# zhoujun-7/VPHO

Hardware: AMD Instinct MI355X
Metric: eval images/sec (bs=64, sample_num=100, steps=50); MPJPE delta vs ref (higher is better)
Workload: dtype f32; 1 GPU; vpho_net.forward(mode=predict), README eval config (BASELINE.json configs[1]); per_gpu_batch=64, sample_num=100, sampling_steps=50, topk_hand=30, topk_obj=10, crop=256x256, pipeline_depth=3, parallelism=dp1, score_mfma=f32, conv_mfma=f32, winograd_3x3=True

## Files before the change

vpho_amd/csrc/conv_igemm.hip:

```cpp
#include "common.h"
#include "../../include/vpho_hip.h"
#include <cstdlib>
#include <algorithm>

VPHO_STAMP_DECL(conv)

namespace {

#ifndef CONV_ABLATE
#define CONV_ABLATE 0
#endif
constexpr int BK = 32;
constexpr int LDS_LD = BK + 4;
constexpr int GLDS_PRE_MAX = 512;

struct Geo {
    vpho_conv_desc d;
    int M, K, tiles_m, tiles_n, ntiles;
    int w_ld;
    long long x_zs, w_zs, y_zs;
    long long b_zs, r_zs, x2_zs, pre_zs, ru_zs;
    int y_linear, r_linear, vec_epilogue;
    int uni;
    int dbg;
};

__device__ __forceinline__ void advance_group(vpho_conv_desc& d, const Geo& g, const unsigned by) {
    d.x += by * g.x_zs; d.w += by * g.w_zs; d.y += by * g.y_zs;
    if (d.bias) d.bias += by * g.b_zs;
    if (d.res) d.res += by * g.r_zs;
    if (d.x2) d.x2 += by * g.x2_zs;
    if (d.in_scale) { d.in_scale += by * g.pre_zs; d.in_shift += by * g.pre_zs; }
    if (d.res_up) d.res_up += by * g.ru_zs;
}

template <int BM, int BN, int WM, int WN, int VEC>
__global__ __launch_bounds__(64 * WM * WN) void conv_igemm_kernel(const Geo g) {
    constexpr int NT = 64 * WM * WN;
    constexpr int TM = BM / (32 * WM), TN = BN / (32 * WN);
    constexpr int KQN = 8 / VEC;
    constexpr int ROWS = NT / KQN;
    constexpr int A_LD = (BM + ROWS - 1) / ROWS, B_LD = (BN + ROWS - 1) / ROWS;
    constexpr bool A_PART = BM < ROWS, B_PART = BN < ROWS;
    static_assert(TM >= 1 && TN >= 1, "tile too small for the wave layout");
    __shared__ __attribute__((aligned(16))) float smem[2 * (BM + BN) * LDS_LD];

    vpho_conv_desc d = g.d;
    advance_group(d, g, blockIdx.y);
    int per_xcd = gridDim.x >> 3, ntiles = g.ntiles, M_live = g.M;
    if (d.row_map) {
        M_live = min(*d.row_count, g.M);
        ntiles = (M_live + BM - 1) / BM * g.tiles_n;
        per_xcd = (ntiles + 7) >> 3;
        if ((int)(blockIdx.x >> 3) >= per_xcd) return;
    }
    const int lb = (blockIdx.x & 7) * per_xcd + (blockIdx.x >> 3);
    if (lb >= ntiles) return;
    const int tile_n = lb % g.tiles_n, tile_m = lb / g.tiles_n;
    const int m0 = tile_m * BM, n0 = tile_n * BN;

    const int tid = threadIdx.x, lane = tid & 63, wave = tid >> 6;
    const int li = lane & 31, lh = lane >> 5;
    const int wm = wave / WN, wn = wave % WN;
    const int kq = tid % KQN, lrow = tid / KQN;

    long long a_off[A_LD];
// ... 598 lines not shown
            float* R = smem;
            if (lane < V_PER_ROW) {
                *reinterpret_cast<f32x4*>(R + (wave * 4 + 0) * BN + 4 * lane) = st0;
                *reinterpret_cast<f32x4*>(R + (wave * 4 + 1) * BN + 4 * lane) = st1;
                *reinterpret_cast<f32x4*>(R + (wave * 4 + 2) * BN + 4 * lane) = piv;
                *reinterpret_cast<f32x4*>(R + (wave * 4 + 3) * BN + 4 * lane) = f32x4{cnt, cnt, cnt, cnt};
            }
            __syncthreads();
            if (d.bn_x) {
                if (tid < 2 * BN) {
                    const int pl = tid / BN, c = tid - pl * BN;
                    float t = R[pl * BN + c];
#pragma unroll
                    for (int k = 1; k < NWAVES; ++k) t += R[(k * 4 + pl) * BN + c];
                    if (n0 + c < d.Cout) d.stats[((long long)tile_m * BN_STAT_PLANES + pl) * d.Cout + n0 + c] = t;
                }
            } else if (tid < BN) {
                const int c = tid;
                ShiftSums t{R[2 * BN + c], R[c], R[BN + c], R[3 * BN + c]};
#pragma unroll
                for (int k = 1; k < NWAVES; ++k) t = shift_sums_add(t, ShiftSums{R[(k * 4 + 2) * BN + c], R[(k * 4) * BN + c], R[(k * 4 + 1) * BN + c], R[(k * 4 + 3) * BN + c]});
                if (n0 + c < d.Cout) store_bn_row(d.stats + (long long)tile_m * BN_STAT_PLANES * d.Cout + n0 + c, d.Cout, t);
            }
        }
        VPHO_STAMP_AT(4);
        VPHO_STAMP_WRITE(conv, blockIdx.x);
        return;
    }
    const int row_base = m0 + wm * (BM / WM) + 4 * lh, col_base = n0 + wn * (BN / WN) + li;
#pragma unroll
    for (int j = 0; j < TN; ++j) {
        const int col = col_base + j * 32;
        if (col >= d.Cout) continue;
        const float bv = d.bias ? d.bias[col] : 0.f;
#pragma unroll
        for (int i = 0; i < TM; ++i) {
#pragma unroll
            for (int e = 0; e < 16; ++e) {
                const int row = row_base + i * 32 + (e & 3) + 8 * (e >> 2);
                if (row >= M_live) continue;
                long long yoff, ro;
                offsets(row, yoff, ro);
                float v = acc[i][j][e] + bv;
                if (d.res) v += d.res[ro + col];
                v = v > 0.f ? v : v * d.out_slope;
                if (d.gate) v = d.gate[yoff + col] > 0.f ? v : v * d.gate_slope;
                d.y[yoff + col] = v;
            }
        }
    }
}

#define VPHO_WAIT_VM(n) asm volatile("s_waitcnt vmcnt(%0)" :: "n"(n) : "memory")
template <int BM, int BN, int WM, int WN, bool STATS>
__device__ __forceinline__ void conv_pers_body(const Geo& g) {
    constexpr int NT = 64 * WM * WN, NW = WM * WN;
    constexpr int TM = BM / (32 * WM), TN = BN / (32 * WN);
    constexpr int ROWS = NT / 8;
    constexpr int A_LD = BM / ROWS, B_LD = BN / ROWS, NF = A_LD + B_LD;
    static_assert(TM >= 1 && TN >= 1 && A_LD >= 1 && B_LD >= 1 && ROWS % 16 == 0 && BN / WN <= 64, "tile/wave layout");
    constexpr int TILE = (BM + BN) * BK;
    constexpr int EPI = 8 * 32;
    constexpr int NIT = TM * 4 * TN;
    __shared__ __attribute__((aligned(1024))) float smem[2 * TILE + NW * EPI + 2 * BN];
    VPHO_STAMP_INIT();

    vpho_conv_desc d = g.d;
    advance_group(d, g, blockIdx.y);
    const int tid = threadIdx.x, lane = tid & 63, wave = __builtin_amdgcn_readfirstlane(tid >> 6);
    const int li = lane & 31, lh = lane >> 5;
    const int wm = wave / WN, wn = wave % WN;
    const int lrow = wave * 8 + (lane >> 3);
    const int kq = (lane & 7) ^ ((lrow >> 1) & 7);
    const int ohw = d.OH * d.OW;
    const __amdgpu_buffer_rsrc_t xu = __builtin_amdgcn_make_buffer_rsrc(const_cast<float*>(d.x), 0, 0xFFFFFFF0u, 0x00020000);
    const __amdgpu_buffer_rsrc_t wr = __builtin_amdgcn_make_buffer_rsrc(const_cast<float*>(d.w), 0, 0xFFFFFFF0u, 0x00020000);
    const __amdgpu_buffer_rsrc_t x2r = __builtin_amdgcn_make_buffer_rsrc(const_cast<float*>(d.x2 ? d.x2 : d.x), 0, 0xFFFFFFF0u, 0x00020000);
    const __amdgpu_buffer_rsrc_t yr = __builtin_amdgcn_make_buffer_rsrc(d.y, 0, 0xFFFFFFF0u, 0x00020000);
    const __amdgpu_buffer_rsrc_t rr = __builtin_amdgcn_make_buffer_rsrc(const_cast<float*>(d.res ? d.res : d.y), 0, 0xFFFFFFF0u, 0x00020000);
    const __amdgpu_buffer_rsrc_t br = __builtin_amdgcn_make_buffer_rsrc(const_cast<float*>(d.bias ? d.bias : d.w), 0, 0xFFFFFFF0u, 0x00020000);
    typedef __attribute__((address_space(3))) void* lds_ptr;

    const int xcd = blockIdx.x & 7, nslot = gridDim.x >> 3, per_xcd = (g.ntiles + 7) >> 3;
    int lt = blockIdx.x >> 3;
    auto tile_at = [&](int t, int& m0, int& n0) -> bool {
        const int lb = xcd * per_xcd + t;
        if (t >= per_xcd || lb >= g.ntiles) return false;
        const int tile_m = lb / g.tiles_n, tile_n = lb - tile_m * g.tiles_n;
        m0 = tile_m * BM; n0 = tile_n * BN;
        return true;
    };
    int m0, n0;
    if (!tile_at(lt, m0, n0)) return;

    int u_voff[A_LD], u_boff[B_LD], u_voff2[A_LD], bias_off;
    auto setup = [&](int m0_, int n0_) {
#pragma unroll
        for (int j = 0; j < A_LD; ++j) {
            const int m = m0_ + lrow + ROWS * j;
            u_voff[j] = -1; u_voff2[j] = -1;
            if (m < g.M) {
                const int n = m / ohw, rem = m - n * ohw;
                const int oy = rem / d.OW, ox = rem - oy * d.OW;
                u_voff[j] = (int)((((long long)(n * d.H + oy * d.stride) * d.W + ox * d.stride) * d.x_ld) * 4 + 16 * kq);
                if (d.x2) u_voff2[j] = (int)((((long long)(n * d.H2 + oy * d.stride2) * d.W2 + ox * d.stride2) * d.x2_ld) * 4 + 16 * kq);
            }
        }
#pragma unroll
        for (int j = 0; j < B_LD; ++j) {
            const int n = n0_ + lrow + ROWS * j;
            u_boff[j] = n < d.Cout ? (int)(((long long)n * g.w_ld + 4 * kq) * 4) : -1;
        }
        const int bc = n0_ + wn * (BN / WN) + lane;
        bias_off = (d.bias && lane < BN / WN && bc < d.Cout) ? bc * 4 : -1;
    };
    auto fill = [&](int buf, int kt, int tp) {
        float* As = smem + buf * TILE + wave * 8 * BK;
        float* Bs = smem + buf * TILE + BM * BK + wave * 8 * BK;
        if (d.x2 && kt * BK >= d.Cin) {
            const int c2 = (kt * BK - d.Cin) * 4;
#pragma unroll
            for (int j = 0; j < A_LD; ++j) {
                const int vo = u_voff2[j];
                __builtin_amdgcn_raw_ptr_buffer_load_lds(x2r, (lds_ptr)(As + ROWS * j * BK), 16, vo, c2, 0, 0);
            }
        } else {
            const int c1 = kt * BK * 4;
#pragma unroll
            for (int j = 0; j < A_LD; ++j) {
                const int vo = u_voff[j];
                __builtin_amdgcn_raw_ptr_buffer_load_lds(xu, (lds_ptr)(As + ROWS * j * BK), 16, vo, c1, 0, 0);
            }
        }
        const int koff = kt * BK * 4;
#pragma unroll
        for (int j = 0; j < B_LD; ++j) {
            const int bo = u_boff[j];
            __builtin_amdgcn_raw_ptr_buffer_load_lds(wr, (lds_ptr)(Bs + ROWS * j * BK), 16, bo, koff, 0, 0);
        }
        if (kt == 0) {
            const int bo = bias_off;
            __builtin_amdgcn_raw_ptr_buffer_load_lds(br, (lds_ptr)(smem + 2 * TILE + NW * EPI + tp * BN + wn * (BN / WN)), 4, bo, 0, 0, 0);
        }
    };

    const int nk = (g.K + BK - 1) / BK;
    const int sw = (li >> 1) & 7;
    f32x16 acc[TM][TN];
    auto compute = [&](int kt) {
        const int buf = kt & 1;
        const float* As = smem + buf * TILE + (wm * (BM / WM) + li) * BK;
        const float* Bs = smem + buf * TILE + BM * BK + (wn * (BN / WN) + li) * BK;
#pragma unroll
        for (int kk = 0; kk < BK / 8; ++kk) {
            const int ch = ((2 * kk + lh) ^ sw) * 4;
            f32x4 a[TM], b[TN];
#pragma unroll
            for (int i = 0; i < TM; ++i) a[i] = *reinterpret_cast<const f32x4*>(As + i * 32 * BK + ch);
#pragma unroll
            for (int j = 0; j < TN; ++j) b[j] = *reinterpret_cast<const f32x4*>(Bs + j * 32 * BK + ch);
#pragma unroll
            for (int q = 0; q < 4; ++q)
#pragma unroll
                for (int i = 0; i < TM; ++i)
#pragma unroll
                    for (int j = 0; j < TN; ++j)
                        acc[i][j] = __builtin_amdgcn_mfma_f32_32x32x2f32(a[i][q], b[j][q], acc[i][j], 0, 0, 0);
        }
    };

    float* Cw = smem + 2 * TILE + wave * EPI;
    const int er = lane >> 3, ec = (lane & 7) * 4;
    auto item_off = [&](int m0_, int n0_, int i, int gq, int j, int& yo, int& ro) {
        const int row = m0_ + wm * (BM / WM) + i * 32 + 8 * gq + er, col = n0_ + wn * (BN / WN) + j * 32 + ec;
        yo = ro = -1;
        if (row < g.M && col < d.Cout) {
            long long y_, r_;
            if (g.y_linear && g.r_linear) { y_ = (long long)row * d.y_sx; r_ = (long long)row * d.r_sx; }
            else {
                const int n = row / ohw, rem = row - n * ohw;
                const int oy = rem / d.OW, ox = rem - oy * d.OW;
                y_ = n * d.y_sn + oy * d.y_sy + ox * d.y_sx; r_ = n * d.r_sn + oy * d.r_sy + ox * d.r_sx;
            }
            yo = (int)((y_ + col) * 4);
            if (d.res) ro = (int)((r_ + col) * 4);
        }
    };

    constexpr bool stats_on = STATS;
    static_assert(4 * (BN / WN) <= EPI && BN <= NT, "stats layout");
    auto flush_stats = [&](int m0_, int n0_) {
        if (tid < BN) {
            const int c = tid;
            const int wn_c = c / (BN / WN), cc = c - wn_c * (BN / WN);
            const float* q = smem + 2 * TILE + wn_c * EPI + cc;
            constexpr int PL = BN / WN;
            ShiftSums t{q[2 * PL], q[0], q[PL], q[3 * PL]};
#pragma unroll
            for (int w = 1; w < WM; ++w) {
                const float* r = q + w * WN * EPI;
                t = shift_sums_add(t, ShiftSums{r[2 * PL], r[0], r[PL], r[3 * PL]});
            }
            if (n0_ + c < d.Cout) store_bn_row(d.stats + (long long)(m0_ / BM) * BN_STAT_PLANES * d.Cout + n0_ + c, d.Cout, t);
        }
    };
    int pm0 = 0, pn0 = 0;

    int tp = 0;
    setup(m0, n0);
    fill(0, 0, tp);
    if (nk > 1) fill(1, 1, tp);
    VPHO_STAMP_AT(1);
    bool first = true;
    while (true) {
        if (nk > 1) { if (first) VPHO_WAIT_VM(NF); else VPHO_WAIT_VM(NF + NIT); }
        else        { if (first) VPHO_WAIT_VM(0);  else VPHO_WAIT_VM(NIT); }
        VPHO_BARRIER_LDS_ONLY();
        if (stats_on && !first) flush_stats(pm0, pn0);
        if (first) VPHO_STAMP_AT(2);
        VPHO_PRIO_MAIN();
#pragma unroll
        for (int i = 0; i < TM; ++i)
#pragma unroll
            for (int j = 0; j < TN; ++j)
#pragma unroll
                for (int e = 0; e < 16; ++e) acc[i][j][e] = 0.f;
        for (int kt = 0; kt + 1 < nk; ++kt) {
            if (kt > 0) fill((kt & 1) ^ 1, kt + 1, tp);
            compute(kt);
            VPHO_SYNC_LDS_DMA();
        }
        f32x4 rv[NIT];
#pragma unroll
        for (int i = 0; i < TM; ++i)
#pragma unroll
            for (int gq = 0; gq < 4; ++gq)
#pragma unroll
                for (int j = 0; j < TN; ++j) {
                    int yo, ro;
                    item_off(m0, n0, i, gq, j, yo, ro);
                    rv[(i * 4 + gq) * TN + j] = __builtin_bit_cast(f32x4, __builtin_amdgcn_raw_buffer_load_b128(rr, ro, 0, 0));
                }
        __builtin_amdgcn_sched_barrier(0);
        compute(nk - 1);
        VPHO_SYNC_LDS_DMA();
#pragma unroll
        for (int k = 0; k < NIT; ++k) asm volatile("" :: "v"(rv[k]));
        VPHO_PRIO_REST();
        if (first) VPHO_STAMP_AT(3);
        const int em0 = m0, en0 = n0, etp = tp;
        lt += nslot;
        const bool more = tile_at(lt, m0, n0);
        if (more) {
            tp ^= 1;
            setup(m0, n0);
            fill(0, 0, tp);
            if (nk > 1) fill(1, 1, tp);
        }
        const float* Bq = smem + 2 * TILE + NW * EPI + etp * BN + wn * (BN / WN) + ec;
        f32x4 st0[TN], st1[TN], piv[TN];
#pragma unroll
        for (int j = 0; j < TN; ++j) { st0[j] = f32x4{0.f, 0.f, 0.f, 0.f}; st1[j] = st0[j]; piv[j] = st0[j]; }
#pragma unroll
        for (int i = 0; i < TM; ++i)
#pragma unroll
            for (int gq = 0; gq < 4; ++gq)
#pragma unroll
                for (int j = 0; j < TN; ++j) {
#pragma unroll
                    for (int e4 = 0; e4 < 4; ++e4) Cw[(e4 + 4 * lh) * 32 + li] = acc[i][j][4 * gq + e4];
                    int yo, ro;
                    item_off(em0, en0, i, gq, j, yo, ro);
                    const f32x4 v = *reinterpret_cast<const f32x4*>(Cw + er * 32 + ec);
                    const f32x4 bq = *reinterpret_cast<const f32x4*>(Bq + j * 32);
                    const f32x4 r = rv[(i * 4 + gq) * TN + j];
                    f32x4 o;
#pragma unroll
                    for (int k = 0; k < 4; ++k) { const float t = v[k] + bq[k] + r[k]; o[k] = t > 0.f ? t : t * d.out_slope; }
                    __builtin_amdgcn_raw_buffer_store_b128(__builtin_bit_cast(__attribute__((__vector_size__(4 * sizeof(unsigned)))) unsigned, o), yr, yo, 0, 0);
                    if (stats_on) {
                        if (i == 0 && gq == 0) {
#pragma unroll
                            for (int k = 0; k < 4; ++k) piv[j][k] = __shfl(o[k], lane & 7);
                        }
#pragma unroll
                        for (int k = 0; k < 4; ++k) { const float u = yo != -1 ? o[k] - piv[j][k] : 0.f; st0[j][k] += u; st1[j][k] += u * u; }
                    }
                }
        if (stats_on) {
            const float n = (float)max(0, min(BM / WM, g.M - (em0 + wm * (BM / WM))));
            static_assert(TM * 32 == BM / WM, "a wave's rows are one block");
#pragma unroll
            for (int j = 0; j < TN; ++j) {
#pragma unroll
                for (int k = 0; k < 4; ++k) { st0[j][k] = sum_lane_bits_345(st0[j][k]); st1[j][k] = sum_lane_bits_345(st1[j][k]); }
                if (lane < 8) {
                    *reinterpret_cast<f32x4*>(Cw + j * 32 + ec) = st0[j];
                    *reinterpret_cast<f32x4*>(Cw + (BN / WN) + j * 32 + ec) = st1[j];
                    *reinterpret_cast<f32x4*>(Cw + 2 * (BN / WN) + j * 32 + ec) = piv[j];
                    *reinterpret_cast<f32x4*>(Cw + 3 * (BN / WN) + j * 32 + ec) = f32x4{n, n, n, n};
                }
            }
            pm0 = em0; pn0 = en0;
        }
        if (first) { VPHO_STAMP_AT(4); }
        first = false;
        if (!more) break;
    }
    if (stats_on) { VPHO_BARRIER_LDS_ONLY(); flush_stats(pm0, pn0); }
    VPHO_STAMP_WRITE(conv, blockIdx.x);
}
template <int BM, int BN, int WM, int WN>
__global__ __launch_bounds__(64 * WM * WN, 4) void conv_igemm_pers_kernel(const Geo g) { conv_pers_body<BM, BN, WM, WN, false>(g); }
template <int BM, int BN, int WM, int WN>
__global__ __launch_bounds__(64 * WM * WN, 4) void conv_igemm_pers_bn_kernel(const Geo g) { conv_pers_body<BM, BN, WM, WN, true>(g); }

typedef __bf16 cbf16x8 __attribute__((ext_vector_type(8)));
constexpr int SBK = 16;

__device__ __forceinline__ void conv_split3(const f32x4& x0, const f32x4& x1, cbf16x8& h, cbf16x8& m, cbf16x8& l) {
#pragma unroll
    for (int e = 0; e < 8; ++e) {
        const float x = e < 4 ? x0[e] : x1[e - 4];
        const __bf16 hb = (__bf16)x;
        const float r1 = x - (float)hb;
        const __bf16 mb = (__bf16)r1;
        const float r2 = r1 - (float)mb;
        h[e] = hb; m[e] = mb; l[e] = (__bf16)r2;
    }
}

template <int BM, int BN, int WM, int WN, int TERMS>
__global__ __launch_bounds__(64 * WM * WN) void conv_igemm_split_kernel(const Geo g) {
    constexpr int NT = 64 * WM * WN, NW = WM * WN;
    constexpr int TM = BM / (32 * WM), TN = BN / (32 * WN);
    constexpr int A_ROWS = NW * 16;
    constexpr int A_LD = BM / A_ROWS;
    constexpr int B_ROWS = NW * 32;
    constexpr int B_PASSES = (3 * BN + B_ROWS - 1) / B_ROWS;
    static_assert(TM >= 1 && TN >= 1 && A_LD >= 1 && BM % A_ROWS == 0, "tile/wave layout");
    constexpr int A_FLOATS = BM * SBK, PLANE_FLOATS = BN * SBK / 2;
    constexpr int TILE = A_FLOATS + 3 * PLANE_FLOATS;
    constexpr int EPI_FLOATS = BM * BN;
    __shared__ __attribute__((aligned(1024))) float smem[(2 * TILE > EPI_FLOATS) ? 2 * TILE : EPI_FLOATS];

    vpho_conv_desc d = g.d;
    int per_xcd = gridDim.x >> 3, ntiles = g.ntiles, M_live = g.M;
    if (d.row_map) {
        M_live = min(*d.row_count, g.M);
        ntiles = (M_live + BM - 1) / BM * g.tiles_n;
        per_xcd = (ntiles + 7) >> 3;
        if ((int)(blockIdx.x >> 3) >= per_xcd) return;
    }
    const int lb = (blockIdx.x & 7) * per_xcd + (blockIdx.x >> 3);
    if (lb >= ntiles) return;
    const int tile_n = lb % g.tiles_n, tile_m = lb / g.tiles_n;
    const int m0 = tile_m * BM, n0 = tile_n * BN;

    const int tid = threadIdx.x, lane = tid & 63, wave = __builtin_amdgcn_readfirstlane(tid >> 6);
    const int li = lane & 31, lh = lane >> 5;
    const int wm = wave / WN, wn = wave % WN;
    const int ohw = d.OH * d.OW;

    const long long pad_shift = ((long long)d.pad_y * d.W + d.pad_x) * d.x_ld;
    const __amdgpu_buffer_rsrc_t xu = __builtin_amdgcn_make_buffer_rsrc(
        reinterpret_cast<void*>(reinterpret_cast<uintptr_t>(d.x) - (uintptr_t)(pad_shift * 4)), 0, 0xFFFFFFF0u, 0x00020000);
    const int arow = wave * 16 + (lane >> 2);
    int a_iy0[A_LD], a_ix0[A_LD], u_voff[A_LD];
// ... 265 lines not shown
                if (d.bn_x && d.bn_gamma) g.d.gate = nullptr;
            } else {
                g.d.stats = nullptr;
                if (d.bn_x) { if (!d.gate) { stats_failed = true; return; } g.d.bn_x = nullptr; }
            }
        }
        hipLaunchKernelGGL(kernel, dim3((g.ntiles + 7) / 8 * 8, ny), dim3(threads), 0, s, g);
    };
    static const int no_glds = getenv("VPHO_CONV_NO_GLDS") ? atoi(getenv("VPHO_CONV_NO_GLDS")) : 0;
    const double x_extent = 4.0 * (((double)d.N * d.H * d.W - 1) * d.x_ld + d.Cin + (double)(ny - 1) * (double)g.x_zs);
    const double w_extent = 4.0 * (((double)d.Cout - 1) * g.w_ld + g.K + (double)(ny - 1) * (double)g.w_zs);
    VPHO_REQUIRE(x_extent < 3.9e9 && w_extent < 3.9e9 && g.x_zs >= 0 && g.w_zs >= 0,
                 "vpho_conv2d_nhwc_f32: input (%.2f GB) and weights (%.2f GB) must each stay below 3.9 GB", x_extent * 1e-9, w_extent * 1e-9);
    static const int no_uni = getenv("VPHO_CONV_NO_UNI") ? atoi(getenv("VPHO_CONV_NO_UNI")) : 0;
    g.uni = (d.Cin % BK == 0 && d.pad_y >= 0 && d.pad_x >= 0 && !no_uni) ? 1 : 0;
    const bool pre_on_read = d.in_scale != nullptr && g.uni && d.KH == 1 && d.KW == 1 && d.pad_y == 0 && d.pad_x == 0 && d.Cin <= GLDS_PRE_MAX;
    const bool glds = (d.in_scale == nullptr || pre_on_read) && (!no_glds || d.res_up != nullptr || d.x2 != nullptr || d.bn_x != nullptr);
    stats_kernel = glds && variant != 128;
    VPHO_REQUIRE(!d.x2 || (g.uni && variant != 128), "vpho_conv2d_nhwc_f32: x2 is served by the direct-to-LDS kernels with wave-uniform taps only");
    VPHO_REQUIRE(!d.res_up || variant != 128, "vpho_conv2d_nhwc_f32: res_up is not served by the forced register-staged tile");
    const bool split_ok = d.w_planes != nullptr && (d.plane_terms == 6 || d.plane_terms == 9) && d.in_scale == nullptr && splits == 1 && !d.gate &&
                          d.Cin % SBK == 0 && g.vec_epilogue && d.pad_y >= 0 && d.pad_x >= 0 && g.w_ld == g.K &&
                          ((uintptr_t)d.w_planes & 15) == 0 && 6.0 * d.Cout * g.K < 3.9e9;
    if (split_ok) {
        const bool x9 = d.plane_terms == 9;
        switch (variant) {
            case 128: case 1288:
                if (x9) launch(conv_igemm_split_kernel<128, 128, 4, 2, 9>, 128, 128, 512, vpho::PROF_CONV128);
                else    launch(conv_igemm_split_kernel<128, 128, 4, 2, 6>, 128, 128, 512, vpho::PROF_CONV128);
                break;
            case 12864:
                if (x9) launch(conv_igemm_split_kernel<128, 64, 4, 2, 9>, 128, 64, 512, vpho::PROF_CONV128x64);
                else    launch(conv_igemm_split_kernel<128, 64, 4, 2, 6>, 128, 64, 512, vpho::PROF_CONV128x64);
                break;
            default:
                if (x9) launch(conv_igemm_split_kernel<64, 64, 2, 2, 9>, 64, 64, 256, vpho::PROF_CONV64);
                else    launch(conv_igemm_split_kernel<64, 64, 2, 2, 6>, 64, 64, 256, vpho::PROF_CONV64);
                break;
        }
        return vpho::check_launch("conv_igemm_split_kernel");
    }
    {
        const char* pe = getenv("VPHO_CONV_PERS");
        const int pers = pe ? atoi(pe) : 1;
        static int slots_of[64] = {0};
        int dev = 0;
        VPHO_HIP(hipGetDevice(&dev));
        int& slots = slots_of[dev & 63];
        if (!slots) {
            hipDeviceProp_t prop;
            VPHO_HIP(hipGetDeviceProperties(&prop, dev));
            slots = 2 * prop.multiProcessorCount;
        }
        const double y_extent = 4.0 * ((double)(d.N - 1) * d.y_sn + (double)(d.OH - 1) * d.y_sy + (double)(d.OW - 1) * d.y_sx + d.Cout);
        const double r_extent = d.res ? 4.0 * ((double)(d.N - 1) * d.r_sn + (double)(d.OH - 1) * d.r_sy + (double)(d.OW - 1) * d.r_sx + d.Cout) : 0.0;
        const bool simple = d.KH == 1 && d.KW == 1 && d.pad_y == 0 && d.pad_x == 0;
        const bool ok = pers && variant == 1288 && glds && !pre_on_read && d.in_scale == nullptr && g.uni && simple && g.vec_epilogue && !d.row_map && !d.res_up &&
                        !d.gate && !d.bn_x && splits == 1 && y_extent < 3.9e9 && r_extent < 3.9e9 && d.y_sn >= 0 && d.y_sy >= 0 && d.y_sx >= 0 &&
                        (!d.x2 || 4.0 * d.N * d.H2 * d.W2 * (double)d.x2_ld < 3.9e9);
        if (ok && (big_tiles > slots || pers >= 2)) {
            vpho::ProfScope prof(vpho::PROF_CONV128, s, flops, bytes);
            g.tiles_m = (int)((M + 127) / 128); g.tiles_n = (d.Cout + 127) / 128;
            g.ntiles = g.tiles_m * g.tiles_n;
            if (d.stats) {
                if (stats_shape && g.tiles_m <= d.stats_cap) *d.stats_rows = g.tiles_m; else g.d.stats = nullptr;
            }
            const int grid = (int)std::min<long long>((g.ntiles + 7) / 8 * 8, std::max(8, slots / groups / 8 * 8));
            if (g.d.stats) hipLaunchKernelGGL((conv_igemm_pers_bn_kernel<128, 128, 4, 2>), dim3(grid, groups), dim3(512), 0, s, g);
            else hipLaunchKernelGGL((conv_igemm_pers_kernel<128, 128, 4, 2>), dim3(grid, groups), dim3(512), 0, s, g);
            return vpho::check_launch("conv_igemm_pers_kernel");
        }
    }
    switch (variant) {
        case 128:  launch(conv_igemm_kernel<128, 128, 2, 2, 1>, 128, 128, 256, vpho::PROF_CONV128); break;
        case 1288:
            if (glds && pre_on_read) launch(conv_igemm_glds_kernel<128, 128, 4, 2, true>, 128, 128, 512, vpho::PROF_CONV128);
            else if (glds) launch(conv_igemm_glds_kernel<128, 128, 4, 2>, 128, 128, 512, vpho::PROF_CONV128);
            else      launch(conv_igemm_kernel<128, 128, 4, 2, 1>, 128, 128, 512, vpho::PROF_CONV128);
            break;
        case 12864:
            if (glds && pre_on_read) launch(conv_igemm_glds_kernel<128, 64, 4, 2, true>, 128, 64, 512, vpho::PROF_CONV128x64);
            else if (glds) launch(conv_igemm_glds_kernel<128, 64, 4, 2>, 128, 64, 512, vpho::PROF_CONV128x64);
            else      launch(conv_igemm_kernel<128, 64, 4, 2, 1>, 128, 64, 512, vpho::PROF_CONV128x64);
            break;
        default:
            if (glds && pre_on_read) launch(conv_igemm_glds_kernel<64, 64, 2, 2, true>, 64, 64, 256, vpho::PROF_CONV64);
            else if (glds) launch(conv_igemm_glds_kernel<64, 64, 2, 2>, 64, 64, 256, vpho::PROF_CONV64);
            else      launch(conv_igemm_kernel<64, 64, 2, 2, 1>, 64, 64, 256, vpho::PROF_CONV64);
            break;
    }
    if (stats_failed)
        return vpho::fail("vpho_conv2d_nhwc_f32: bn_x: the launch needs %d partial rows (stats_cap %d) or runs a kernel without the BatchNorm epilogue (tile %d)",
                          g.tiles_m, d.stats_cap, variant);
    return vpho::check_launch("conv_igemm_kernel");
}
```

vpho_amd/ops.py:

```python
import ctypes as C
import os

import torch

_HERE = os.path.dirname(os.path.abspath(__file__))
LIB_PATH = os.environ.get('VPHO_HIP_LIB') or os.path.join(_HERE, 'libvpho_hip.so')

if not os.path.exists(LIB_PATH):
    raise ImportError(f'{LIB_PATH} is missing: build the HIP extension first (python -m vpho_amd.build or '
                      f'__graft_entry__.build()); vpho_amd has no CPU fallback')
lib = C.CDLL(LIB_PATH)
lib.vpho_last_error.restype = C.c_char_p
lib.vpho_abi_version.restype = C.c_int
ABI_VERSION = 13
if lib.vpho_abi_version() != ABI_VERSION:
    raise ImportError(f'{LIB_PATH} implements ABI version {lib.vpho_abi_version()}, this binding expects {ABI_VERSION}: rebuild the '
                      f'extension (python -m vpho_amd.build --force)')
lib.vpho_obj_metrics_workspace_bytes.restype = C.c_longlong
lib.vpho_obj_metrics_multi_workspace_bytes.restype = C.c_longlong
lib.vpho_bn_workspace_bytes.restype = C.c_longlong
lib.vpho_conv2d_wgrad_workspace_bytes.restype = C.c_longlong
lib.vpho_mha_bwd_workspace_bytes.restype = C.c_longlong
lib.vpho_infer_record_bytes.restype = C.c_longlong
lib.vpho_hand_obj_intersection_workspace_bytes.restype = C.c_longlong
# ... 114 lines not shown
            assert N % G == 0, (N, G)
            N //= G
    cin = x_ld if cin is None else cin
    cout = w.shape[-2]
    assert split is not None or w.shape[-1] == kh * kw * cin + (0 if x2 is None else x2.shape[-1]), (w.shape, kh, kw, cin)
    py = pad if pad_y is None else pad_y
    px = pad if pad_x is None else pad_x
    if out_hw is None:
        OH, OW = (H + 2 * py - kh) // stride + 1, (W + 2 * px - kw) // stride + 1
    else:
        OH, OW = out_hw
    d = ConvDesc()
    d.x, d.w, d.bias = _addr(x), _addr(w), _addr(bias)
    d.in_scale, d.in_shift, d.res = _addr(in_scale), _addr(in_shift), _addr(res)
    for t in (x, w, bias, in_scale, in_shift, res):
        _ptr(t, torch.float32)
    if rows is not None:
        assert out_view is None and res is None and gate is None and rows.shape == (N, OH, OW) and (res_up is None or rows_scatter)
        if out is None:
            out = torch.empty((N, OH, OW, cout) if rows_scatter else (N * OH * OW, cout), device=x.device, dtype=torch.float32)
        _ptr(out, torch.float32)
        ld = out.shape[-1]
        d.y, d.y_sx, d.y_sy, d.y_sn = out.data_ptr(), ld, (ld * OW if rows_scatter else 0), (ld * OW * OH if rows_scatter else 0)
        d.rows_scatter = 1 if rows_scatter else 0
        d.row_map, d.row_count = rows.row_map.data_ptr(), rows.count.data_ptr()
        d.rows_hint = int(rows.count.item()) if _prof_on else 0
        ret = out
    elif out_view is not None:
        yt, d.y_sn, d.y_sy, d.y_sx, off = out_view
        _ptr(yt, torch.float32)
        d.y = yt.data_ptr() + 4 * off
        ret = yt
        if gate is not None:
            assert gate[0].shape == yt.shape and gate[0].is_contiguous() and yt.is_contiguous()
            d.gate, d.gate_slope = _ptr(gate[0], torch.float32).value + 4 * off, gate[1]
    else:
        if out is None:
            out = torch.empty((G * N, OH, OW, cout), device=x.device, dtype=torch.float32)
        _ptr(out, torch.float32)
        assert out.shape[0] == G * N
        ld = out.shape[-1]
        d.y, d.y_sx, d.y_sy, d.y_sn = out.data_ptr(), ld, ld * OW, ld * OW * OH
        ret = out
        if gate is not None:
            assert gate[0].shape == out.shape
            d.gate, d.gate_slope = _ptr(gate[0], torch.float32).value, gate[1]
    if res is not None:
        assert res.shape == (G * N, OH, OW, cout)
        d.r_sx, d.r_sy, d.r_sn = cout, cout * OW, cout * OW * OH
    if x2 is not None:
        assert kh == kw == 1 and rows is None and split is None and in_scale is None and x2.shape[0] == (N if (G == 1 or x2_shared) else G * N) and x2.is_contiguous()
        d.x2, d.Cin2, d.x2_ld, d.stride2, d.H2, d.W2 = _ptr(x2, torch.float32).value, x2.shape[3], x2.shape[3], stride2, x2.shape[1], x2.shape[2]
    if res_up is not None:
        assert res is None and res_up.shape[0] == G * N and res_up.shape[3] == cout and res_up.is_contiguous()
        d.res_up, d.ru_H, d.ru_W, d.ru_ld = _ptr(res_up, torch.float32).value, res_up.shape[1], res_up.shape[2], res_up.shape[3]
    if G > 1:
        assert in_scale is None or (in_scale.shape == (G, cin) and in_shift.shape == (G, cin) and in_scale.is_contiguous() and in_shift.is_contiguous())
        d.groups = G
        d.x_group = 0 if x_shared else N * H * W * x_ld
        d.w_group, d.bias_group, d.y_group = w.shape[1] * w.shape[2], cout, (ret.numel() // G if out_view is not None else N * OH * OW * ret.shape[-1])
        d.res_group = N * OH * OW * cout
        d.x2_group = 0 if (x2 is None or x2_shared) else N * x2.shape[1] * x2.shape[2] * x2.shape[3]
        d.pre_group = cin
        d.ru_group = 0 if res_up is None else N * res_up.shape[1] * res_up.shape[2] * res_up.shape[3]
    d.N, d.H, d.W, d.Cin, d.x_ld = N, H, W, cin, x_ld
    d.Cout, d.KH, d.KW, d.stride, d.pad_y, d.pad_x, d.OH, d.OW = cout, kh, kw, stride, py, px, OH, OW
    d.in_slope, d.out_slope = in_slope, out_slope
    if split is not None:
        d.splits, d.w_ld, d.x_split, d.w_split, d.y_split = split
    terms = getattr(_conv_split, 'terms', 0)
    if terms and G == 1 and split is None and in_scale is None and gate is None and res_up is None and x2 is None and cin % 16 == 0 and w.is_contiguous() and w.shape[1] == kh * kw * cin:
        planes = _planes_of(w)
        d.w_planes, d.plane_terms = planes.data_ptr(), terms
    rows_out = None
    if bn is not None and FUSE_BN and G == 1 and split is None and rows is None and in_scale is None and (out_view is None or bn.parts > 1) and not d.w_planes and cout % 4 == 0:
        cap = (N * OH * OW + 63) // 64
        if bn.stats is None:
            bn.stats = torch.empty((cap * bn.parts, BN_STAT_PLANES, cout), device=x.device, dtype=torch.float32)
        base = bn.rows
        assert base + cap <= bn.stats.shape[0] and bn.stats.shape[2] == cout
        rows_out = C.c_int(0)
        d.stats, d.stats_cap, d.stats_rows = bn.stats.data_ptr() + base * BN_STAT_PLANES * cout * 4, cap, C.cast(C.pointer(rows_out), C.c_void_p)
        if bn.x is not None:
            assert gate is not None and bn.x.shape == ret.shape and bn.x.is_contiguous() and ret.is_contiguous()
            bx = _ptr(bn.x, torch.float32).value + (4 * out_view[4] if out_view is not None else 0)
            if bn.stored_gate:
                d.bn_x, d.bn_mean, d.bn_invstd = bx, _ptr(bn.mean, torch.float32).value, _ptr(bn.invstd, torch.float32).value
            else:
                d.bn_x = bx
                d.bn_mean, d.bn_invstd, d.bn_gamma, d.bn_beta = (_ptr(t, torch.float32).value for t in (bn.mean, bn.invstd, bn.gamma, bn.beta))
    elif bn is not None:
        bn.failed = True
    _check(lib.vpho_conv2d_nhwc_f32(C.byref(d), _stream()))
    if rows_out is not None:
        bn.calls += 1
        if rows_out.value == 0:
            bn.failed = True
        bn.rows += rows_out.value
    return ret


def conv3x3(x, w, bias=None, out_slope=1.0, winograd=True, rows=None, groups=1, x_shared=False):
    N, H, W, x_ld = x.shape
    cout, k9 = w.shape[-2:]
    cin = k9 // 9
    if not winograd or H % 2 or W % 2 or cin % 16 or cout % 64 or x_ld != cin:
        return conv2d_nhwc(x, w, bias, kh=3, kw=3, pad=1, out_slope=out_slope, rows=rows, groups=groups, x_shared=x_shared)
# ... 1351 lines not shown
```

Measured before the change: 2104 images/s.

## Route row-gathered and upsampled-residual 1x1 convs through persistent 128x64 kernel

Adds a GATHER variant of the persistent implicit-GEMM conv body. It reads a row map (pixel list) and a bilinear-upsampled residual, precomputing per-row output and residual offsets into an LDS record. The upsampled-residual loads are interleaved with the final K iterations. It also enables a 128x64 narrow-tile persistent path for variant 12864, so those convs leave the non-persistent kernels. The cost is extra LDS, more complex epilogue and index code, and a relaxed res_up channel assertion.

```diff
diff --git a/vpho_amd/csrc/conv_igemm.hip b/vpho_amd/csrc/conv_igemm.hip
--- a/vpho_amd/csrc/conv_igemm.hip
+++ b/vpho_amd/csrc/conv_igemm.hip
@@ -12,6 +12,7 @@
 #endif
 constexpr int BK = 32;
 constexpr int LDS_LD = BK + 4;
+constexpr bool PERS_DEFAULT_GATHER = true, PERS_DEFAULT_NARROW = true;
 constexpr int GLDS_PRE_MAX = 512;
 
 struct Geo {
@@ -716,8 +717,9 @@
 }
 
 #define VPHO_WAIT_VM(n) asm volatile("s_waitcnt vmcnt(%0)" :: "n"(n) : "memory")
-template <int BM, int BN, int WM, int WN, bool STATS>
+template <int BM, int BN, int WM, int WN, bool STATS, bool GATHER = false>
 __device__ __forceinline__ void conv_pers_body(const Geo& g) {
+    static_assert(!(STATS && GATHER), "the BatchNorm epilogue takes no pixel list / up-sampled residual");
     constexpr int NT = 64 * WM * WN, NW = WM * WN;
     constexpr int TM = BM / (32 * WM), TN = BN / (32 * WN);
     constexpr int ROWS = NT / 8;
@@ -726,7 +728,10 @@
     constexpr int TILE = (BM + BN) * BK;
     constexpr int EPI = 8 * 32;
     constexpr int NIT = TM * 4 * TN;
-    __shared__ __attribute__((aligned(1024))) float smem[2 * TILE + NW * EPI + 2 * BN];
+    constexpr int BIAS_AT = BN / WN == 64 ? 64 : 0;
+    static_assert(BN / WN == 64 || BN == 64, "bias fill: one dword per lane");
+    constexpr int REC = GATHER ? 32 * 4 : 0;
+    __shared__ __attribute__((aligned(1024))) float smem[2 * TILE + NW * EPI + 2 * BN + NW * REC];
     VPHO_STAMP_INIT();
 
     vpho_conv_desc d = g.d;
@@ -743,13 +748,20 @@
     const __amdgpu_buffer_rsrc_t yr = __builtin_amdgcn_make_buffer_rsrc(d.y, 0, 0xFFFFFFF0u, 0x00020000);
     const __amdgpu_buffer_rsrc_t rr = __builtin_amdgcn_make_buffer_rsrc(const_cast<float*>(d.res ? d.res : d.y), 0, 0xFFFFFFF0u, 0x00020000);
     const __amdgpu_buffer_rsrc_t br = __builtin_amdgcn_make_buffer_rsrc(const_cast<float*>(d.bias ? d.bias : d.w), 0, 0xFFFFFFF0u, 0x00020000);
+    const __amdgpu_buffer_rsrc_t rur = __builtin_amdgcn_make_buffer_rsrc(const_cast<float*>(GATHER && d.res_up ? d.res_up : d.w), 0, 0xFFFFFFF0u, 0x00020000);
+    const __amdgpu_buffer_rsrc_t mr = __builtin_amdgcn_make_buffer_rsrc(GATHER && d.row_map ? (void*)const_cast<int*>(d.row_map) : (void*)const_cast<float*>(d.w), 0, 0xFFFFFFF0u, 0x00020000);
     typedef __attribute__((address_space(3))) void* lds_ptr;
-
-    const int xcd = blockIdx.x & 7, nslot = gridDim.x >> 3, per_xcd = (g.ntiles + 7) >> 3;
+    int m_live = g.M, nt_live = g.ntiles;
+    if constexpr (GATHER) {
+        if (d.row_map) { m_live = min(*d.row_count, g.M); nt_live = (m_live + BM - 1) / BM * g.tiles_n; }
+    }
+    const int M_live = GATHER ? m_live : g.M, ntiles = GATHER ? nt_live : g.ntiles;
+
+    const int xcd = blockIdx.x & 7, nslot = gridDim.x >> 3, per_xcd = (ntiles + 7) >> 3;
     int lt = blockIdx.x >> 3;
     auto tile_at = [&](int t, int& m0, int& n0) -> bool {
         const int lb = xcd * per_xcd + t;
-        if (t >= per_xcd || lb >= g.ntiles) return false;
+        if (t >= per_xcd || lb >= ntiles) return false;
         const int tile_m = lb / g.tiles_n, tile_n = lb - tile_m * g.tiles_n;
         m0 = tile_m * BM; n0 = tile_n * BN;
         return true;
@@ -757,17 +769,71 @@
     int m0, n0;
     if (!tile_at(lt, m0, n0)) return;
 
+    int ar[A_LD], erow[TM];
+    auto rows_of = [&](int m0_, bool have) {
+#pragma unroll
+        for (int j = 0; j < A_LD; ++j) {
+            const int m = m0_ + lrow + ROWS * j;
+            const bool live = have && m < M_live;
+            int v = m;
+            if (d.row_map) v = __builtin_amdgcn_raw_buffer_load_b32(mr, live ? m * 4 : -1, 0, 0);
+            ar[j] = live ? v : -1;
+        }
+#pragma unroll
+        for (int i = 0; i < TM; ++i) {
+            const int m = m0_ + wm * (BM / WM) + i * 32 + li;
+            const bool live = have && m < M_live;
+            int v = m;
+            if (d.row_map) v = __builtin_amdgcn_raw_buffer_load_b32(mr, live ? m * 4 : -1, 0, 0);
+            erow[i] = live ? v : -1;
+        }
+    };
+    int* const Rw = reinterpret_cast<int*>(smem + 2 * TILE + NW * EPI + 2 * BN + wave * REC);
+    typedef int i32x4 __attribute__((ext_vector_type(4)));
+    i32x4 rec_next = {-1, -1, 0, 0};
+    auto make_rec = [&](int m0_) {
+        const float sy = (float)d.ru_H / (float)d.OH, sx = (float)d.ru_W / (float)d.OW;
+#pragma unroll
+        for (int i = 0; i < TM; ++i) {
+            static_assert(!GATHER || TM == 1, "one record block per wave");
+            const int pix = erow[i];
+            int ry = -1, ro_ = -1;
+            float ly = 0.f, lx = 0.f;
+            if (pix >= 0) {
+                const int n = pix / ohw, rem = pix - n * ohw;
+                const int oy = rem / d.OW, ox = rem - oy * d.OW;
+                long long y_, r_;
+                if (g.y_linear && g.r_linear) {
+                    const int orow = (d.row_map && !d.rows_scatter) ? m0_ + wm * (BM / WM) + i * 32 + li : pix;
+                    y_ = (long long)orow * d.y_sx; r_ = (long long)orow * d.r_sx;
+                } else { y_ = n * d.y_sn + oy * d.y_sy + ox * d.y_sx; r_ = n * d.r_sn + oy * d.r_sy + ox * d.r_sx; }
+                ry = (int)(y_ * 4);
+                if (d.res) ro_ = (int)(r_ * 4);
+                if (d.res_up) {
+                    int y0, y1, x0, x1;
+                    lin_src(oy, sy, d.ru_H, y0, y1, ly);
+                    lin_src(ox, sx, d.ru_W, x0, x1, lx);
+                    ro_ = (int)((((long long)n * d.ru_H + y0) * d.ru_W + x0) * d.ru_ld * 4) | (x1 != x0 ? 1 : 0) | (y1 != y0 ? 2 : 0);
+                }
+            }
+            rec_next = i32x4{ry, ro_, __builtin_bit_cast(int, ly), __builtin_bit_cast(int, lx)};
+        }
+    };
+    auto put_rec = [&]() { *reinterpret_cast<i32x4*>(Rw + 4 * li) = rec_next; };
+
     int u_voff[A_LD], u_boff[B_LD], u_voff2[A_LD], bias_off;
     auto setup = [&](int m0_, int n0_) {
 #pragma unroll
         for (int j = 0; j < A_LD; ++j) {
-            const int m = m0_ + lrow + ROWS * j;
+            int m = m0_ + lrow + ROWS * j;
             u_voff[j] = -1; u_voff2[j] = -1;
-            if (m < g.M) {
+            bool live = m < M_live;
+            if constexpr (GATHER) { m = ar[j]; live = m >= 0; }
+            if (live) {
                 const int n = m / ohw, rem = m - n * ohw;
                 const int oy = rem / d.OW, ox = rem - oy * d.OW;
                 u_voff[j] = (int)((((long long)(n * d.H + oy * d.stride) * d.W + ox * d.stride) * d.x_ld) * 4 + 16 * kq);
-                if (d.x2) u_voff2[j] = (int)((((long long)(n * d.H2 + oy * d.stride2) * d.W2 + ox * d.stride2) * d.x2_ld) * 4 + 16 * kq);
+                if (!GATHER && d.x2) u_voff2[j] = (int)((((long long)(n * d.H2 + oy * d.stride2) * d.W2 + ox * d.stride2) * d.x2_ld) * 4 + 16 * kq);
             }
         }
 #pragma unroll
@@ -775,13 +841,13 @@
             const int n = n0_ + lrow + ROWS * j;
             u_boff[j] = n < d.Cout ? (int)(((long long)n * g.w_ld + 4 * kq) * 4) : -1;
         }
-        const int bc = n0_ + wn * (BN / WN) + lane;
-        bias_off = (d.bias && lane < BN / WN && bc < d.Cout) ? bc * 4 : -1;
+        const int bc = n0_ + BIAS_AT * wn + lane;
+        bias_off = (d.bias && bc < n0_ + BN && bc < d.Cout) ? bc * 4 : -1;
     };
     auto fill = [&](int buf, int kt, int tp) {
         float* As = smem + buf * TILE + wave * 8 * BK;
         float* Bs = smem + buf * TILE + BM * BK + wave * 8 * BK;
-        if (d.x2 && kt * BK >= d.Cin) {
+        if (!GATHER && d.x2 && kt * BK >= d.Cin) {
             const int c2 = (kt * BK - d.Cin) * 4;
 #pragma unroll
             for (int j = 0; j < A_LD; ++j) {
@@ -804,7 +870,7 @@
         }
         if (kt == 0) {
             const int bo = bias_off;
-            __builtin_amdgcn_raw_ptr_buffer_load_lds(br, (lds_ptr)(smem + 2 * TILE + NW * EPI + tp * BN + wn * (BN / WN)), 4, bo, 0, 0, 0);
+            __builtin_amdgcn_raw_ptr_buffer_load_lds(br, (lds_ptr)(smem + 2 * TILE + NW * EPI + tp * BN + BIAS_AT * wn), 4, bo, 0, 0, 0);
         }
     };
 
@@ -817,7 +883,12 @@
         const float* Bs = smem + buf * TILE + BM * BK + (wn * (BN / WN) + li) * BK;
 #pragma unroll
         for (int kk = 0; kk < BK / 8; ++kk) {
-            const int ch = ((2 * kk + lh) ^ sw) * 4;
+            int ch = ((2 * kk + lh) ^ sw) * 4;
+            if constexpr (GATHER) {
+                int sel = 8 * kk;
+                asm volatile("" : "+v"(sel));
+                ch = ((lh ^ sw) * 4) ^ sel;
+            }
             f32x4 a[TM], b[TN];
 #pragma unroll
             for (int i = 0; i < TM; ++i) a[i] = *reinterpret_cast<const f32x4*>(As + i * 32 * BK + ch);
@@ -838,6 +909,11 @@
     auto item_off = [&](int m0_, int n0_, int i, int gq, int j, int& yo, int& ro) {
         const int row = m0_ + wm * (BM / WM) + i * 32 + 8 * gq + er, col = n0_ + wn * (BN / WN) + j * 32 + ec;
         yo = ro = -1;
+        if constexpr (GATHER) {
+            const int yb = Rw[4 * (8 * gq + er)], rb = Rw[4 * (8 * gq + er) + 1];
+            if (yb != -1 && col < d.Cout) { yo = yb + col * 4; if (d.res) ro = rb + col * 4; }
+            return;
+        }
         if (row < g.M && col < d.Cout) {
             long long y_, r_;
             if (g.y_linear && g.r_linear) { y_ = (long long)row * d.y_sx; r_ = (long long)row * d.r_sx; }
@@ -870,7 +946,31 @@
     };
     int pm0 = 0, pn0 = 0;
 
+    f32x4 rv[NIT], tc[4];
+    auto ru_issue = [&](int q, int n0_) {
+        const int gq = (q / TN) & 3, j = q % TN;
+        const int col = n0_ + wn * (BN / WN) + j * 32 + ec;
+        const int o = Rw[4 * (8 * gq + er) + 1];
+        const bool live = o != -1 && col < d.Cout;
+        const int dx = (o & 1) ? d.ru_ld * 4 : 0, dy = (o & 2) ? d.ru_W * d.ru_ld * 4 : 0;
+        const int o00 = live ? (o & ~3) + col * 4 : -1, o01 = live ? o00 + dx : -1, o10 = live ? o00 + dy : -1, o11 = live ? o10 + dx : -1;
+        tc[0] = __builtin_bit_cast(f32x4, __builtin_amdgcn_raw_buffer_load_b128(rur, o00, 0, 0));
+        tc[1] = __builtin_bit_cast(f32x4, __builtin_amdgcn_raw_buffer_load_b128(rur, o01, 0, 0));
+        tc[2] = __builtin_bit_cast(f32x4, __builtin_amdgcn_raw_buffer_load_b128(rur, o10, 0, 0));
+        tc[3] = __builtin_bit_cast(f32x4, __builtin_amdgcn_raw_buffer_load_b128(rur, o11, 0, 0));
+    };
+    auto ru_combine = [&](int q) {
+        const int gq = (q / TN) & 3;
+        const float ly = __builtin_bit_cast(float, Rw[4 * (8 * gq + er) + 2]), lx = __builtin_bit_cast(float, Rw[4 * (8 * gq + er) + 3]);
+        const float hy = 1.f - ly, hx = 1.f - lx;
+#pragma unroll
+        for (int u = 0; u < 4; ++u) rv[q][u] = hy * (hx * tc[0][u] + lx * tc[1][u]) + ly * (hx * tc[2][u] + lx * tc[3][u]);
+    };
+    const int ru_first = max(0, nk - 1 - NIT);
+    (void)rows_of; (void)make_rec; (void)put_rec; (void)ru_issue; (void)ru_combine; (void)ru_first;
+
     int tp = 0;
+    if constexpr (GATHER) { rows_of(m0, true); make_rec(m0); put_rec(); }
     setup(m0, n0);
     fill(0, 0, tp);
     if (nk > 1) fill(1, 1, tp);
@@ -891,10 +991,25 @@
                 for (int e = 0; e < 16; ++e) acc[i][j][e] = 0.f;
         for (int kt = 0; kt + 1 < nk; ++kt) {
             if (kt > 0) fill((kt & 1) ^ 1, kt + 1, tp);
+            if constexpr (GATHER) {
+                if (d.res_up && kt >= ru_first) {
+#pragma unroll
+                    for (int q = 0; q < NIT; ++q) if (q == kt - ru_first) ru_issue(q, n0);
+                }
+            }
             compute(kt);
             VPHO_SYNC_LDS_DMA();
-        }
-        f32x4 rv[NIT];
+            if constexpr (GATHER) {
+                if (d.res_up && kt >= ru_first) {
+#pragma unroll
+                    for (int q = 0; q < NIT; ++q) if (q == kt - ru_first) ru_combine(q);
+                }
+            }
+        }
+        if (GATHER && d.res_up) {
+#pragma unroll
+            for (int q = 0; q < NIT; ++q) if (q >= nk - 1 - ru_first) { ru_issue(q, n0); ru_combine(q); }
+        } else {
 #pragma unroll
         for (int i = 0; i < TM; ++i)
 #pragma unroll
@@ -905,11 +1020,23 @@
                     item_off(m0, n0, i, gq, j, yo, ro);
                     rv[(i * 4 + gq) * TN + j] = __builtin_bit_cast(f32x4, __builtin_amdgcn_raw_buffer_load_b128(rr, ro, 0, 0));
                 }
+        }
+        if constexpr (GATHER) {
+            int nm0 = 0, nn0 = 0;
+            const bool have = tile_at(lt + nslot, nm0, nn0);
+            rows_of(nm0, have);
+        }
         __builtin_amdgcn_sched_barrier(0);
         compute(nk - 1);
         VPHO_SYNC_LDS_DMA();
 #pragma unroll
         for (int k = 0; k < NIT; ++k) asm volatile("" :: "v"(rv[k]));
+        if constexpr (GATHER) {
+#pragma unroll
+            for (int i = 0; i < TM; ++i) asm volatile("" :: "v"(erow[i]));
+#pragma unroll
+            for (int j = 0; j < A_LD; ++j) asm volatile("" :: "v"(ar[j]));
+        }
         VPHO_PRIO_REST();
         if (first) VPHO_STAMP_AT(3);
         const int em0 = m0, en0 = n0, etp = tp;
@@ -917,6 +1044,7 @@
         const bool more = tile_at(lt, m0, n0);
         if (more) {
             tp ^= 1;
+            if constexpr (GATHER) make_rec(m0);
             setup(m0, n0);
             fill(0, 0, tp);
             if (nk > 1) fill(1, 1, tp);
@@ -970,6 +1098,7 @@
         if (first) { VPHO_STAMP_AT(4); }
         first = false;
         if (!more) break;
+        if constexpr (GATHER) put_rec();
     }
     if (stats_on) { VPHO_BARRIER_LDS_ONLY(); flush_stats(pm0, pn0); }
     VPHO_STAMP_WRITE(conv, blockIdx.x);
@@ -978,6 +1107,8 @@
 __global__ __launch_bounds__(64 * WM * WN, 4) void conv_igemm_pers_kernel(const Geo g) { conv_pers_body<BM, BN, WM, WN, false>(g); }
 template <int BM, int BN, int WM, int WN>
 __global__ __launch_bounds__(64 * WM * WN, 4) void conv_igemm_pers_bn_kernel(const Geo g) { conv_pers_body<BM, BN, WM, WN, true>(g); }
+template <int BM, int BN, int WM, int WN>
+__global__ __launch_bounds__(64 * WM * WN, 4) void conv_igemm_pers_gather_kernel(const Geo g) { conv_pers_body<BM, BN, WM, WN, false, true>(g); }
 
 typedef __bf16 cbf16x8 __attribute__((ext_vector_type(8)));
 constexpr int SBK = 16;
@@ -1349,21 +1480,32 @@
             VPHO_HIP(hipGetDeviceProperties(&prop, dev));
             slots = 2 * prop.multiProcessorCount;
         }
-        const double y_extent = 4.0 * ((double)(d.N - 1) * d.y_sn + (double)(d.OH - 1) * d.y_sy + (double)(d.OW - 1) * d.y_sx + d.Cout);
-        const double r_extent = d.res ? 4.0 * ((double)(d.N - 1) * d.r_sn + (double)(d.OH - 1) * d.r_sy + (double)(d.OW - 1) * d.r_sx + d.Cout) : 0.0;
+        const bool compact = d.row_map && !d.rows_scatter;
+        const double y_extent = compact ? 4.0 * ((double)(M - 1) * d.y_sx + d.Cout)
+                                        : 4.0 * ((double)(d.N - 1) * d.y_sn + (double)(d.OH - 1) * d.y_sy + (double)(d.OW - 1) * d.y_sx + d.Cout);
+        const double r_extent = !d.res ? 0.0 : compact ? 4.0 * ((double)(M - 1) * d.r_sx + d.Cout)
+                                        : 4.0 * ((double)(d.N - 1) * d.r_sn + (double)(d.OH - 1) * d.r_sy + (double)(d.OW - 1) * d.r_sx + d.Cout);
         const bool simple = d.KH == 1 && d.KW == 1 && d.pad_y == 0 && d.pad_x == 0;
-        const bool ok = pers && variant == 1288 && glds && !pre_on_read && d.in_scale == nullptr && g.uni && simple && g.vec_epilogue && !d.row_map && !d.res_up &&
+        const bool gather = d.row_map != nullptr || d.res_up != nullptr;
+        const bool narrow = variant == 12864 || (gather && variant == 1288);
+        const bool ok = pers && (variant == 1288 || variant == 12864) && glds && !pre_on_read && d.in_scale == nullptr && g.uni && simple && g.vec_epilogue &&
                         !d.gate && !d.bn_x && splits == 1 && y_extent < 3.9e9 && r_extent < 3.9e9 && d.y_sn >= 0 && d.y_sy >= 0 && d.y_sx >= 0 &&
-                        (!d.x2 || 4.0 * d.N * d.H2 * d.W2 * (double)d.x2_ld < 3.9e9);
-        if (ok && (big_tiles > slots || pers >= 2)) {
-            vpho::ProfScope prof(vpho::PROF_CONV128, s, flops, bytes);
-            g.tiles_m = (int)((M + 127) / 128); g.tiles_n = (d.Cout + 127) / 128;
+                        (!d.x2 || 4.0 * d.N * d.H2 * d.W2 * (double)d.x2_ld < 3.9e9) &&
+                        !((gather || narrow) && d.stats) && !(gather && d.x2) && (!d.row_map || 4.0 * (double)M < 3.9e9);
+        const bool by_default = gather ? PERS_DEFAULT_GATHER : (narrow ? PERS_DEFAULT_NARROW : true);
+        const long long tiles = narrow ? tiles_12864 : big_tiles;
+        if (ok && ((tiles > slots && by_default) || pers >= 2)) {
+            const int bn = narrow ? 64 : 128;
+            vpho::ProfScope prof(narrow ? vpho::PROF_CONV128x64 : vpho::PROF_CONV128, s, flops, bytes);
+            g.tiles_m = (int)((M + 127) / 128); g.tiles_n = (d.Cout + bn - 1) / bn;
             g.ntiles = g.tiles_m * g.tiles_n;
             if (d.stats) {
                 if (stats_shape && g.tiles_m <= d.stats_cap) *d.stats_rows = g.tiles_m; else g.d.stats = nullptr;
             }
             const int grid = (int)std::min<long long>((g.ntiles + 7) / 8 * 8, std::max(8, slots / groups / 8 * 8));
-            if (g.d.stats) hipLaunchKernelGGL((conv_igemm_pers_bn_kernel<128, 128, 4, 2>), dim3(grid, groups), dim3(512), 0, s, g);
+            if (gather) hipLaunchKernelGGL((conv_igemm_pers_gather_kernel<128, 64, 4, 2>), dim3(grid, groups), dim3(512), 0, s, g);
+            else if (narrow) hipLaunchKernelGGL((conv_igemm_pers_kernel<128, 64, 4, 2>), dim3(grid, groups), dim3(512), 0, s, g);
+            else if (g.d.stats) hipLaunchKernelGGL((conv_igemm_pers_bn_kernel<128, 128, 4, 2>), dim3(grid, groups), dim3(512), 0, s, g);
             else hipLaunchKernelGGL((conv_igemm_pers_kernel<128, 128, 4, 2>), dim3(grid, groups), dim3(512), 0, s, g);
             return vpho::check_launch("conv_igemm_pers_kernel");
         }
diff --git a/vpho_amd/ops.py b/vpho_amd/ops.py
--- a/vpho_amd/ops.py
+++ b/vpho_amd/ops.py
@@ -190,7 +190,7 @@
         assert kh == kw == 1 and rows is None and split is None and in_scale is None and x2.shape[0] == (N if (G == 1 or x2_shared) else G * N) and x2.is_contiguous()
         d.x2, d.Cin2, d.x2_ld, d.stride2, d.H2, d.W2 = _ptr(x2, torch.float32).value, x2.shape[3], x2.shape[3], stride2, x2.shape[1], x2.shape[2]
     if res_up is not None:
-        assert res is None and res_up.shape[0] == G * N and res_up.shape[3] == cout and res_up.is_contiguous()
+        assert res is None and res_up.shape[0] == G * N and res_up.shape[3] >= cout and res_up.is_contiguous()
         d.res_up, d.ru_H, d.ru_W, d.ru_ld = _ptr(res_up, torch.float32).value, res_up.shape[1], res_up.shape[2], res_up.shape[3]
     if G > 1:
         assert in_scale is None or (in_scale.shape == (G, cin) and in_shift.shape == (G, cin) and in_scale.is_contiguous() and in_shift.is_contiguous())
```

Result: no change. 2097 images/s (-0.3%).
